# sony/DiffRoll

Measured on AMD Instinct MI355X. Metric: piano-roll frames/sec (200-step sample), higher is better.
Workload: dtype f32

## Files before the change

### diffroll_amd/csrc/abi.hip

```cpp
#include "engine_state.h"
#include "tenants.h"

#include <algorithm>
#include <condition_variable>
#include <mutex>

namespace drh {

thread_local std::string g_create_error;
void release_stager(int dev);
std::atomic<int> g_engines[MAX_DEVICES];

struct FusedSlot {
    std::mutex mu;
    std::condition_variable cv;
    dr_engine* owner = nullptr;
    bool claimed = false;
    hipEvent_t done = nullptr;
};
FusedSlot g_slots[MAX_DEVICES];

bool claim_fused_slot(dr_engine* e, hipStream_t st) {
    FusedSlot& s = g_slots[e->cfg.device];
    std::unique_lock<std::mutex> lk(s.mu);
// ... 377 lines not shown
        return DR_OK;
    }
    if (n == "start_noise") {
        if (value != 0 && value != 1)
            return fail(e, DR_EINVAL, "start_noise is 0 (x on entry is x at the start step) or 1 (a clean roll, diffused to it), got %d", value);
        e->opt.start_noise = value;
        return DR_OK;
    }
    if (n == "x0_clip") {
        if (value < 0 || value > 2)
            return fail(e, DR_EINVAL, "x0_clip is 0 (off), 1 (clamp the x0 prediction to [0, 1]) or 2 (to [-1, 1]), got %d", value);
        if (e->opt.x0_clamp != value) e->hist_key.valid = false;
        e->opt.x0_clamp = value;
        return DR_OK;
    }
    if (n == "x0_threshold") {
        if (value != 0 && (value < 5000 || value > 10000))
            return fail(e, DR_EINVAL, "x0_threshold is 0 (off) or the percentile in units of 1 / 10000, 5000 .. 10000 (9950 = 99.5 %%), got %d", value);
        if (e->opt.x0_thresh != value) e->hist_key.valid = false;
        e->opt.x0_thresh = value;
        return DR_OK;
    }
    if (n == "guidance_t_min" || n == "guidance_t_max") {
        const bool is_max = n == "guidance_t_max";
        if (!guidance_value_ok(is_max, value, e->S))
            return fail(e, DR_EINVAL, is_max ? "guidance_t_max is -1 (= timesteps - 1) or in [0, timesteps = %d), got %d"
                                             : "guidance_t_min is in [0, timesteps = %d), got %d", e->S, value);
        (is_max ? e->opt.guid.hi : e->opt.guid.lo) = value;
        return DR_OK;
    }
    if (!lab) return fail(e, DR_ENAME, "unknown option '%s'", name);
    if (n == "fused_stack_xcd") { if (e->opt_stack_xcd != value) drop(); e->opt_stack_xcd = value; return DR_OK; }
    if (n == "fused_stack_warm") { if (e->opt_stack_warm != value) drop(); e->opt_stack_warm = value; return DR_OK; }
#ifdef DR_FAULT_HOOK
    if (n == "stack_fault_test") { if (e->opt_stack_fault != value) drop(); e->opt_stack_fault = value; return DR_OK; }
#endif
    if (n == "stack_ticks") { if (e->stack_dbg_on != value) drop(); e->stack_dbg_on = value; return DR_OK; }
    if (n.compare(0, 5, "tune.") == 0) {
        Tuning& t = tuning();
        const std::string f = n.substr(5);
        if (f == "ksplit_blocks") {
            if (t.ksplit_blocks.load() != value) { t.ksplit_blocks.store(value); tuning_epoch().fetch_add(1); drop(); }
            return DR_OK;
        }
        std::atomic<int>* field = f == "pack_threads" ? &t.pack_threads : f == "tile" ? &t.tile : f == "pw" ? &t.pw : f == "pw_nw" ? &t.pw_nw
                   : f == "pwk" ? &t.pwk : f == "ksplit_max" ? &t.ksplit_max : f == "one_ks" ? &t.one_ks : f == "stack3" ? &t.stack3
                   : f == "stack_fl" ? &t.stack_fl : f == "tail_t4" ? &t.tail_t4 : f == "xcd_n" ? &t.xcd_n : f == "xcd_model" ? &t.xcd_model
                   : f == "s3_eager" ? &t.s3_eager : f == "debug_chunks" ? &t.debug_chunks : nullptr;
        if (!field) return fail(e, DR_ENAME, "unknown option '%s'", name);
        if (field->load() != value) {
            field->store(value);
            tuning_epoch().fetch_add(1);
            drop();
        }
        return DR_OK;
    }
    return fail(e, DR_ENAME, "unknown option '%s'", name);
}

int open_chain_call(dr_engine* e, int sampler, int B, int T, const int* step, int& NB, int& i0, hipStream_t st) {
    int rc = check_ready(e, sampler, B, T);
    if (rc) return rc;
    if (step) {
        const int t = *step;
        if (t < 0 || t >= e->S) return fail(e, DR_EINVAL, "step %d out of range", t);
        if (!e->rs_steps.empty() && std::find(e->rs_steps.begin(), e->rs_steps.end(), t) == e->rs_steps.end())
// ... 503 lines not shown
```

### diffroll_amd/csrc/engine_state.h

```cpp
#pragma once
#include <hip/hip_runtime.h>

#include <dlfcn.h>

#include <atomic>
#include <chrono>
#include <cmath>
#include <cstdarg>
#include <cstdio>
#include <cstdlib>
#include <cstring>
#include <map>
#include <memory>
#include <string>
#include <thread>
#include <vector>

#include "../../include/diffroll_amd_debug.h"
#include "device_buffer.h"
#include "fused_mode.h"
#include "kernels.h"

namespace drh {
using namespace dr;
// ... 113 lines not shown

    int ws_NB = 0, ws_T = 0;
    drh::DevBuf<float> sk_ws;
    drh::DevBuf<unsigned> sk_cnt;
    drh::DevBuf<float> h, hd, g, skip, tmp, x0buf;
    drh::DevBuf<float> xwork;
    drh::DevBuf<float> hd3, g3;
    int prec = 0;
    bool s3_ready = false;
    double t_pack_s = 0.0, t_upload_s = 0.0, t_tables_s = 0.0, t_capture_s = 0.0;
    int norm_framewise = 0;
    int fe_B = 0, fe_T = 0;
    drh::DevBuf<float> cond;
    drh::DevBuf<float> cond_dummy;
    drh::DevBuf<float> cond_tr;
    int cond_tr_T = 0;
    drh::DevBuf<float> wav_pad, power, logmel, specP4, mm;

    drh::GraphKey gkey;
    hipGraph_t graph = nullptr;
    hipGraphExec_t gexec = nullptr;
    drh::DevBuf<long long> dbg_ticks;
    drh::DevBuf<unsigned long long> d_counts;
    size_t mm_scratch_off = 0;
    hipStream_t cap_stream = nullptr;
    drh::DevBuf<dr::DynParams> d_dyn;
    drh::DevBuf<int> d_tsel;
    bool use_dyn = false;

    drh::FusedMode fused;
    int opt_stack_xcd = 1;
    int opt_stack_fault = 0;
    int opt_stack_warm = 0;
    int n_cus = 0;
    drh::StackSync sync;
    int opt_tail = 1;
    int64_t tail_launches = 0;
    drh::ChainOptions opt;
    std::vector<int> win_marks;
    drh::DevBuf<unsigned> d_wintab;
    std::vector<int> rs_steps;
    drh::DevBuf<float> d_coef_rs;
    std::vector<float> h_solver;
    drh::DevBuf<float> d_solver;
    drh::DevBuf<float> hist;
    int hist_par = 0;
    struct { bool valid = false; int sampler = -1, B = 0, T = 0, t = -1; } hist_key;
    drh::DevBuf<unsigned> thresh_work;
    int64_t inproj_launches = 0;
    int64_t conv0_launches = 0;
    unsigned win_epoch = 0;
    drh::DevBuf<float> xalt;
    int last_mode = 0;
    unsigned tuning_epoch = 0;
    long kfd_gpu_id = -1;
    double last_tenant_scan_s = -1.0;
    hipStream_t graph_stream = nullptr;
    bool graph_stream_set = false;
    bool unverified = false;
    hipStream_t fused_stream = nullptr;
    int opt_blocked = 2;
    drh::DevBuf<float> xsave;
    drh::DevBuf<long long> stack_dbg;
    int stack_dbg_on = 0;
    int64_t stack_launches = 0;

// ... 123 lines not shown
```

### diffroll_amd/csrc/gemm_body.h

```cpp
#pragma once
#include "device_common.h"

namespace dr {

DR_DEVINL void residual_quad(const float (&v)[4], const float4 bias, const float4 prev, float (&o)[4]) {
    float bb[4], pv[4];
    f4arr(bias, bb); f4arr(prev, pv);
#pragma unroll
    for (int e = 0; e < 4; ++e) o[e] = div_sqrt2(pv[e] + (v[e] + bb[e]));
}
DR_DEVINL void skip_quad(const float (&v)[4], const float4 bias, const float4 prev, const bool skip_init, float (&o)[4]) {
    float bb[4], pv[4];
    f4arr(bias, bb); f4arr(prev, pv);
#pragma unroll
    for (int e = 0; e < 4; ++e) o[e] = skip_init ? v[e] + bb[e] : (v[e] + bb[e]) + pv[e];
}
DR_DEVINL long cond_row(const GemmArgs& a, const int b) {
    int r = a.c_b0 + b;
    if (a.c_n > 0 && r >= a.c_n) r %= a.c_n;
    return r;
}
DR_DEVINL void gate_quad(const float (&v0)[4], const float (&v1)[4], const float4 bias0, const float4 bias1,
                         const float4 cond0, const float4 cond1, const bool has_c, float (&o)[4]) {
    float b0[4], b1[4], c0[4], c1[4];
// ... 16 lines not shown
DR_DEVINL void store_y2(const GemmArgs& a, const int b, const float (&o)[4], const float4 d, const int p0, const int t) {
    float o2[4];
    hd_quad(o, d, o2);
    if (a.out_s3 & 2) {
        store_s3_quad<COH3>(a.Y2 + (long)b * a.y2_bs, o2, p0, t, a.T, a.y_rows >> 3, a.wt_store);
    } else {
        float* dst2 = a.Y2 + (long)b * a.y2_bs + (long)(p0 >> 2) * a.y_ps + (long)t * a.y_fs;
        store_f4<COH4>(dst2, make_float4(o2[0], o2[1], o2[2], o2[3]), a.wt_store);
    }
}

DR_DEVINL AF4 load_a4(const __amdgpu_buffer_rsrc_t wrsrc, const int wvo, const int slab, const int NS, const int code) {
    AF4 o;
#pragma unroll
    for (int g = 0; g < 4; ++g) {
        DR_CHECK(slab >= 0 && wvo + slab * 16384 + g * 4096 + 16 <= NS * 16384, code, slab, NS);
        o.v[g] = buffer_load_f4(wrsrc, wvo, slab * 16384 + g * 4096);
    }
    return o;
}

typedef __attribute__((address_space(3))) void* lds_ptr;

template <int BN, int AUX, class PlaneOf>
DR_DEVINL void dma_tile(float4* Rs, PlaneOf plane_of, const int T, const int t0, const int first, const int stride, const int lane, const int code) {
    constexpr int RWL = (BN + 63) / 64;
    for (int i = first; i < 32 * RWL; i += stride) {
        const int pl = i / RWL, seg = i - pl * RWL;
        const int f = seg * 64 + lane;
        const __amdgpu_buffer_rsrc_t rsrc = __builtin_amdgcn_make_buffer_rsrc((void*)plane_of(pl), 0, (unsigned)T * 16u, 0x00020000);
        if (BN % 64 == 0 || f < BN) {
            DR_CHECK_LDS(Rs + pl * BN + f, lds_off(Rs), lds_off(Rs) + 32u * BN * 16u, code);
            __builtin_amdgcn_raw_ptr_buffer_load_lds(rsrc, (lds_ptr)(Rs + pl * BN + seg * 64), 16, (t0 + f) * 16, 0, 0, AUX);
        }
    }
}

template <int KS, int PREC, int AUX, int RBN>
DR_DEVINL void producer(const GemmArgs& a, float4* Xs, float4* Rs, const int pw, const int lane, const int mt, const int b, const int t0,
                        const int halo, const int FW, const int c0, const int c1, const int code_x, const int code_r) {
    constexpr int XP = (PREC ? 12 : 8) * KS;
    const int bx = a.x_bmod ? (b % a.x_bmod) : b;
    const float* Xg = a.X + (long)bx * a.x_bs;
    const int last_plane = a.x_planes - 1;
    const unsigned recs = ((unsigned)(a.T - 1) * (unsigned)a.x_fs + 4u) * 4u;
    const int wl = (FW + 63) >> 6;
    const int total = XP * wl;
    auto issue = [&](int chunk) {
        for (int i = pw; i < total; i += 4) {
            const int pl = i / wl, seg = i - pl * wl;
            const int f = seg * 64 + lane;
            const float* src;
            if constexpr (PREC) {
                const int sg = pl / 6, rem = pl - sg * 6, pce = rem >> 1, kq = rem & 1;
                const int pc = min(chunk * (4 * KS) + sg * 2 + kq, last_plane);
                src = Xg + (long)pce * a.x_piece + (long)pc * a.x_ps;
            } else {
                src = Xg + (long)min(chunk * XP + pl, last_plane) * a.x_ps;
            }
            const __amdgpu_buffer_rsrc_t rsrc = __builtin_amdgcn_make_buffer_rsrc((void*)src, 0, recs, 0x00020000);
            const int voff = (t0 - halo + f) * (int)a.x_fs * 4;
            float4* dst = Xs + (((chunk - c0) & 1) * XP + pl) * FW + seg * 64;
            if (f < FW) DR_CHECK_LDS(dst + lane, lds_off(Xs), lds_off(Xs) + 2u * XP * FW * 16u, code_x);
            if (f < FW) __builtin_amdgcn_raw_ptr_buffer_load_lds(rsrc, (lds_ptr)dst, 16, voff, 0, 0, AUX);
        }
    };
// ... 411 lines not shown
                        } else {
                            float* dst = a.skip + (long)be * a.s_bs + ((long)((p0 - a.y_rows) >> 2) * a.T + t) * 4;
                            skip_quad(v, ebias[q], eop[ni][q], a.skip_init, o);
                            *reinterpret_cast<float4*>(dst) = make_float4(o[0], o[1], o[2], o[3]);
                        }
                    } else {
                        if (p0 >= a.y_rows) continue;
                        float bb[4];
                        f4arr(ebias[q], bb);
    #pragma unroll
                        for (int e = 0; e < 4; ++e) {
                            if constexpr (EPI == EPI_PLAIN) o[e] = a.alpha * v[e] + bb[e];
                            else if constexpr (EPI == EPI_RELU) o[e] = fmaxf(a.alpha * v[e] + bb[e], 0.f);
                            else if constexpr (EPI == EPI_SILU) { const float z = v[e] + bb[e]; o[e] = z * sigmoidf_(z); }
                            else o[e] = logf(v[e] + 1e-6f);
                        }
                        float* dst = a.Y + (long)be * a.y_bs + (long)(p0 >> 2) * a.y_ps + (long)t * a.y_fs;
                        *reinterpret_cast<float4*>(dst) = make_float4(o[0], o[1], o[2], o[3]);
                        if constexpr (EPI == EPI_RELU) {
                            if (a.Y2) store_y2<COH, 0>(a, be, o, ed2[q], p0, t);
                        }
                    }
                }
            }
        }
    }
    if (a.dbg && blockIdx.x == 0 && tid == 0) {
        a.dbg[0] = tick1 - tick0;
        a.dbg[1] = clock64() - tick0;
    }
}

template <int NW, int COH, int RLDS, int TBN = 32 * NW, int EPI = EPI_RES_SKIP>
DR_DEVINL void pw_body(const GemmArgs& a, const int mt, const int nt, const int wave, float4* Rs = nullptr, const int foff = 0) {
    static_assert(EPI == EPI_RES_SKIP || EPI == EPI_RELU || EPI == EPI_PLAIN, "pw_body epilogues");
    static_assert(EPI == EPI_RES_SKIP || !RLDS, "the LDS-resident tile belongs to the residual / skip epilogue");
    constexpr int BN = TBN;
    int lane = threadIdx.x & 63;
    if constexpr (COH) asm volatile("" : "+v"(lane));
    const int r = lane & 31, hi = lane >> 5;
    const long long tick0 = a.dbg ? clock64() : 0;

    const int tps = (a.T + BN - 1) / BN;
    const int b = nt / tps;
    const int t0 = (nt % tps) * BN + foff;
    const int NS = a.kchunks;

    const __amdgpu_buffer_rsrc_t wr = __builtin_amdgcn_make_buffer_rsrc(
        (void*)(a.Wp + (long)mt * NS * 4096), 0, (unsigned)NS * 16384u, 0x00020000);
    const __amdgpu_buffer_rsrc_t xr = __builtin_amdgcn_make_buffer_rsrc(
        (void*)(a.X + (long)b * a.x_bs), 0, (unsigned)(a.x_planes * a.x_ps * 4), 0x00020000);
    const int wvo = (hi * 128 + wave * 32 + r) * 16;
    const int xps = (int)a.x_ps * 4;
    int xvo[NW];
#pragma unroll
    for (int ni = 0; ni < NW; ++ni) xvo[ni] = hi * xps + min(t0 + ni * 32 + r, a.T - 1) * 16;

    struct BF { float4 v[4][NW]; };
    auto load_a = [&](int slab) { return load_a4(wr, wvo, slab, NS, 120); };
    auto load_b = [&](int slab) -> BF {
        BF o;
#pragma unroll
        for (int g = 0; g < 4; ++g)
#pragma unroll
            for (int ni = 0; ni < NW; ++ni)
                o.v[g][ni] = buffer_load_f4(xr, xvo[ni], (slab * 8 + g * 2) * xps);
        return o;
// ... 36 lines not shown
        for (int q = 0; q < 4; ++q) {
            ebias[q] = *reinterpret_cast<const float4*>(a.bias + rowb + 8 * q);
            if constexpr (EPI == EPI_RES_SKIP)
                ed2[q] = *reinterpret_cast<const float4*>(a.d2 + (a.tsel ? (long)a.tsel[b] * a.d2_ts : 0) + min(rowb + 8 * q, a.y_rows - 4));
        }
        if constexpr (RLDS || EPI != EPI_RES_SKIP) return;
        const float* base = res_rows ? a.Y + (long)b * a.y_bs + (long)(rowb >> 2) * a.y_ps
                                     : a.skip + (long)b * a.s_bs + (long)((rowb - a.y_rows) >> 2) * a.T * 4;
        const long qs = res_rows ? 2 * a.y_ps : (long)2 * a.T * 4;
        const long fs = res_rows ? a.y_fs : 4;
#pragma unroll
        for (int ni = 0; ni < NW; ++ni) {
            const int tc = min(t0 + ni * 32 + r, a.T - 1);
#pragma unroll
            for (int q = 0; q < 4; ++q) eop[ni][q] = *reinterpret_cast<const float4*>(base + q * qs + tc * fs);
        }
    };
    int slab = 0;
    const int pre = max(NS - 2, 0) & ~1;
    for (; slab < pre; slab += 2) {
        step(std::false_type{}, slab);
        step(std::true_type{}, slab + 1);
        if (a.dbg && slab == 0 && blockIdx.x == 0 && threadIdx.x == 0) a.dbg[2] = clock64() - tick0;
    }
    if (a.dbg && blockIdx.x == 0 && threadIdx.x == 0) a.dbg[3] = clock64() - tick0;
    if constexpr (!RLDS) load_epilogue();
    __builtin_amdgcn_sched_barrier(0);
    for (; slab + 2 <= NS; slab += 2) {
        step(std::false_type{}, slab);
        step(std::true_type{}, slab + 1);
    }
    if (slab < NS) step(std::false_type{}, slab);
    const long long tick1 = a.dbg ? clock64() : 0;
    if constexpr (RLDS) load_epilogue();

#pragma unroll
    for (int ni = 0; ni < NW; ++ni) {
        const int t = t0 + ni * 32 + r;
        if (t >= a.T) continue;
#pragma unroll
        for (int q = 0; q < 4; ++q) {
            const int p0 = rowb + 8 * q;
            float v[4], o[4];
#pragma unroll
            for (int e = 0; e < 4; ++e) v[e] = acc[ni][4 * q + e];
            if constexpr (EPI != EPI_RES_SKIP) {
                if (p0 >= a.y_rows) continue;
                float bb[4];
                f4arr(ebias[q], bb);
#pragma unroll
                for (int e = 0; e < 4; ++e) {
                    o[e] = a.alpha * v[e] + bb[e];
                    if constexpr (EPI == EPI_RELU) o[e] = fmaxf(o[e], 0.f);
                }
                float* dst = a.Y + (long)b * a.y_bs + (long)(p0 >> 2) * a.y_ps + (long)t * a.y_fs;
                store_f4<COH>(dst, make_float4(o[0], o[1], o[2], o[3]), a.wt_store);
                continue;
            }
            float4* rs = nullptr;
            if constexpr (RLDS) rs = Rs + (wave * 8 + 2 * q + hi) * BN + foff + ni * 32 + r;
#ifdef DR_BOUNDS
            if constexpr (RLDS) DR_CHECK_LDS(rs, lds_off(Rs), lds_off(Rs) + 32u * BN * 16u, 121);
#endif
            float4 pv;
            if constexpr (RLDS) pv = *rs;
            else pv = eop[ni][q];
            if (res_rows) {
// ... 205 lines not shown
```

### diffroll_amd/csrc/kernels.h

```cpp
#pragma once
#include <hip/hip_runtime.h>
#include <stdint.h>

#include <atomic>

#include "launch_plan.h"

namespace dr {


struct Tuning {
    std::atomic<int> pack_threads{16};
    std::atomic<int> tile{0};
    std::atomic<int> pw{1};
    std::atomic<int> pw_nw{0};
    std::atomic<int> pwk{1};
    std::atomic<int> ksplit_max{16};
    std::atomic<long> ksplit_blocks{0};
    std::atomic<int> one_ks{0};
    std::atomic<int> stack3{1};
    std::atomic<int> stack_fl{0};
    std::atomic<int> tail_t4{0};
    std::atomic<int> xcd_n{-1};
    std::atomic<int> xcd_model{1};
// ... 49 lines not shown
    int wt_store;
};

hipError_t init_kernels();
hipError_t read_bounds(unsigned long long* out4);
hipError_t reset_bounds();
hipError_t launch_gemm(const GemmArgs& a, int epi, int NI, hipStream_t s, int prec = 0);
hipError_t launch_gemm16(const GemmArgs& a, int epi, int NJ, hipStream_t s);
hipError_t launch_pointwise(const GemmArgs& a, int NW, hipStream_t s);
hipError_t launch_pointwise_ksplit(const GemmArgs& a, int NW, hipStream_t s);

struct StackLayer {
    const float *conv_w, *conv_b, *conv_b2;
    const float *cond, *cond2;
    const float *out_w, *out_b;
    int dil, pad_;
};
struct StackArgs {
    float *h, *hd, *g, *skip;
    const float* d2;
    const int* tsel;
    long d2_ts;
    const float* zero;
    int NB, T, Cp, taps, n_cond, L;
    long c_bs;
    int c_b0, c_n;
    int p0, p1;
    int xcd_n;
    int rs_off;
    int lds_bytes;
    int fault;
    int fold128;
    int warm;
    unsigned* xid;
    unsigned* bar;
    unsigned* err;
    unsigned* derr;
    long long* dbg;
    StackLayer layer[DR_STACK_MAX_LAYERS];
};
hipError_t launch_stack(const StackArgs& s, int FL, int max_dil, hipStream_t st, int prec = 0);

struct DynParams {
    unsigned long long seed;
    int first_sample;
    float w, onepw;
    unsigned epoch;
};
hipError_t launch_set_dyn(DynParams* d, unsigned long long seed, int first_sample, float w, float onepw, unsigned epoch,
                          hipStream_t s);

struct UpdateArgs {
    float* x;
    const float* x0c;
    const float* x0u;
    const float* noise;
    const float* coef;
    int t;
    int mode;
    long n;
    long per_sample;
    float w, onepw;
    uint64_t seed;
    int first_sample;
    const DynParams* dyn;
    int win_H;
// ... 84 lines not shown
```

### diffroll_amd/csrc/launch_plan.h

```cpp
#pragma once
#include <algorithm>
#include <cstddef>

#include "../../include/diffroll_amd.h"

namespace dr {

enum Epilogue : int {
    EPI_PLAIN = 0,
    EPI_RELU = 1,
    EPI_SILU = 2,
    EPI_GATE = 3,
    EPI_RES_SKIP = 4,
    EPI_POWER = 5,
    EPI_LOG = 6
};

constexpr int DR_STACK_MAX_LAYERS = 30;
constexpr int STACK_GROUPS = 512;
constexpr size_t SK_WS_FLOATS = (size_t)16 << 20, SK_CNT_N = 4096;

struct PlanKnobs {
    int tile = 0, pw = 1, pw_nw = 0, pwk = 1, ksplit_max = 16;
    long ksplit_blocks = 0;
// ... 10 lines not shown

struct KSplitPlan { int ks; double us; double us_unsplit; };
inline KSplitPlan plan_ksplit(const PlanKnobs& k, long tiles, int nchunks, int kchunks, int taps, int NI, int prec,
                              size_t ws_floats, size_t ws_cnt_n) {
    const int ks_max = k.ksplit_max;
    const long forced_blocks = k.ksplit_blocks;
    const long max_blocks = forced_blocks ? forced_blocks : (prec ? 256 : 2048);
    const int BN = gemm_block_frames(NI);
    const double t_full = (double)kchunks * taps * 16.0 * (BN / 32) * 69.0 / 2400.0;
    auto cost = [&](int ks) {
        return (double)((tiles * ks + 255) / 256) * t_full / ks + (ks > 1 ? 4.0 + ks : 0.0);
    };
    KSplitPlan p{1, cost(1), cost(1)};
    for (int ks = 2; ks <= ks_max && ks <= 16; ks *= 2) {
        if (tiles * ks > max_blocks || nchunks % ks != 0) break;
        if ((size_t)tiles * ks * 128 * BN > ws_floats || (size_t)tiles * 4 > ws_cnt_n) break;
        const double c = cost(ks);
        if (tiles * ks <= 256 || c < 0.97 * p.us) { p.us = std::min(p.us, c); p.ks = ks; }
    }
    return p;
}

inline int stack_tile_frames(int FL) { return FL == 5 ? 160 : 64 * FL; }
inline size_t stack3_lds_bytes(int FL, int taps, int max_dil) {
    return std::max(gemm_lds_bytes(FL, 1, taps, max_dil, 1, EPI_GATE), gemm_lds_bytes(1, 4, 1, 1, 1, EPI_RES_SKIP)) + 16;
}
inline int stack_group_blocks(int FL, int Cp, int T) {
    const int BN = stack_tile_frames(FL);
    return (Cp >> 6) * ((T + BN - 1) / BN);
}
inline size_t stack_lds_bytes(int FL, int taps, int max_dil) {
    const int BN = stack_tile_frames(FL), halo = ((taps - 1) / 2) * max_dil;
    return (size_t)2 * 8 * (BN + 2 * halo) * 16 + (size_t)32 * BN * 16 + 16;
}

struct Tile { int flavor, n; };

inline double split_cost(const PlanKnobs& k, long blocks, int bn, double pen, int MT, int taps) {
    const int nchunks = 2 * MT;
    const KSplitPlan p = plan_ksplit(k, blocks, nchunks, nchunks, taps, bn / 64, 0, SK_WS_FLOATS, SK_CNT_N);
    if (p.ks <= 1 || blocks * p.ks <= 256) return 1e30;
    const double us_per_frame = p.us_unsplit / ((double)((blocks + 255) / 256) * bn);
    return 1.05 * pen * p.us / us_per_frame;
}
inline Tile pick_tile(const PlanKnobs& k, int MT, int NB, int T, int taps, int dil, int prec, int epi, bool allow16,
                      bool wide32 = false) {
    const int forced = k.tile;
    const int halo = ((taps - 1) / 2) * dil;
    struct Cand { int flavor, n, bn; double pen; };
    const Cand cands[] = {{0, 2, 128, 1.0}, {0, 5, 160, 1.04}, {1, 5, 160, 1.04}, {0, 3, 96, 1.04}, {1, 3, 96, 1.04}, {0, 1, 64, 1.0}};
    auto feasible = [&](const Cand& c) {
        if (c.flavor == 1 && (!allow16 || prec != 0)) return false;
        if (c.flavor == 0 && (c.n == 3 || c.n == 5) && (!wide32 || prec != 0 || epi != EPI_GATE || taps == 1)) return false;
        const int ks = (taps == 1) ? 2 : 1;
        const size_t lds = (c.flavor == 0)
            ? gemm_lds_bytes(c.n, (taps == 1 && c.n == 1) ? 4 : ks, taps, dil, prec, epi)
            : (size_t)2 * 8 * ks * (c.bn + 2 * halo) * 16 + (epi == EPI_RES_SKIP ? (size_t)32 * c.bn * 16 : 0);
        return lds <= 160 * 1024;
    };
    if (forced) {
        const int ff = forced / 100 == 16 ? 1 : 0, fn = forced % 100;
        for (const Cand& c : cands)
            if (c.flavor == ff && c.n == fn && feasible(c)) return Tile{ff, fn};
    }
    Tile best{0, 1};
    double best_cost = 1e30;
// ... 125 lines not shown
```

### diffroll_amd/csrc/plan.hip

```cpp
#include "engine_state.h"

namespace drh {

hipError_t launch_tiled(const GemmArgs& a, int epi, Tile t, hipStream_t s, int prec) {
    if (t.flavor == 3) return launch_pointwise_ksplit(a, t.n, s);
    if (t.flavor == 2) return launch_pointwise(a, t.n, s);
    return t.flavor == 1 ? launch_gemm16(a, epi, t.n, s) : launch_gemm(a, epi, t.n, s, prec);
}
void allow_splitk(const dr_engine* e, GemmArgs& a) {
    a.ws = e->sk_ws; a.ws_cnt = e->sk_cnt;
    a.ws_floats = SK_WS_FLOATS; a.ws_cnt_n = SK_CNT_N;
}

const float* g_zero_vecs[MAX_DEVICES] = {};
const float* zero_vec() {
    int dev = 0;
    (void)hipGetDevice(&dev);
    return (dev >= 0 && dev < MAX_DEVICES) ? g_zero_vecs[dev] : nullptr;
}

GemmArgs p4_gemm(const float* Wp, const float* bias, int MT, const float* X, int planes, int NB, int T) {
    GemmArgs a{};
    a.d2 = zero_vec();
    a.Wp = Wp; a.bias = bias ? bias : zero_vec(); a.MT = MT;
// ... 84 lines not shown
    a.X = v.xin; a.x_bs = (long)T * 88; a.x_ps = 4; a.x_fs = 88; a.x_planes = 22; a.x_bmod = v.bmod;
    a.kchunks = 3; a.NB = v.NB; a.T = T; a.taps = 1; a.dil = 1; a.alpha = 1.f;
    p4_out(a, e->h, Cp / 4, T, Cp);
    a.d2 = e->d_dtab + (v.tsel ? 0 : (size_t)v.t * e->L * Cp);
    a.tsel = v.tsel; a.d2_ts = (long)e->L * Cp;
    if (e->prec) { a.Y2 = e->hd3; a.y2_bs = act_bs + act_bs / 2; a.out_s3 = 2; }
    else { a.Y2 = e->hd; a.y2_bs = act_bs; }
    allow_splitk(e, a);
    HIPCHK(e, launch_gemm(a, EPI_RELU, pick_ni(k, a.MT, v.NB, T, 1, 1), v.st));
    e->inproj_launches += 1;
    return DR_OK;
}

static int launch_stack_range(const Eval& v, const NetPlan& p, int p0, int p1) {
    dr_engine* e = v.e;
    const int Cp = e->Cp, L = e->L, T = v.T, prec = e->prec;
    const long act_n = (long)Cp * T, c_bs = (long)2 * Cp * T;
    int b0 = 0;
    for (int ck = 0; ck < p.stack_chunks; ++ck) {
        const int nb = v.NB / p.stack_chunks + (ck < v.NB % p.stack_chunks ? 1 : 0);
        StackArgs sa{};
        sa.h = e->h + b0 * act_n; sa.hd = e->hd + b0 * act_n; sa.g = e->g + b0 * act_n; sa.skip = e->skip + b0 * act_n;
        if (prec) { sa.hd = e->hd3 + b0 * (act_n + act_n / 2); sa.g = e->g3 + b0 * (act_n + act_n / 2); }
        sa.d2 = e->d_dtab + (v.tsel ? 0 : (size_t)v.t * L * Cp);
        sa.tsel = v.tsel ? v.tsel + b0 : nullptr; sa.d2_ts = (long)L * Cp;
        sa.zero = zero_vec();
        sa.NB = nb; sa.T = T; sa.Cp = Cp; sa.taps = e->K; sa.L = L;
        sa.n_cond = std::max(0, std::min(nb, v.n_cond - b0));
        sa.c_bs = c_bs;
        sa.c_b0 = b0 < v.n_cond ? b0 : 0; sa.c_n = e->fe_B;
        sa.p0 = p0; sa.p1 = p1;
        sa.xcd_n = e->opt_stack_xcd;
        sa.warm = e->opt_stack_warm;
        sa.fault = e->opt_stack_fault;
        sa.fold128 = e->opt_blocked >= 2;
        sa.bar = e->sync.bar(); sa.err = e->sync.err; sa.derr = e->sync.derr(); sa.xid = e->sync.xid();
        sa.dbg = e->stack_dbg_on ? e->stack_dbg : nullptr;
        for (int l = 0; l < L; ++l) {
            const LayerW& w = e->layers[l];
            StackLayer& y = sa.layer[l];
            y.conv_w = prec ? w.conv_w3 : w.conv_w; y.conv_b = w.conv_b;
            y.conv_b2 = v.zero_spec ? w.conv_b_z : w.conv_b_u;
            y.cond2 = nullptr;
            if (e->cond_tr && !v.zero_spec) { y.cond2 = e->cond_tr + (size_t)l * 2 * Cp * T; y.conv_b2 = w.conv_b; }
            y.cond = e->cond ? e->cond + (size_t)l * e->fe_B * 2 * Cp * T : e->cond_dummy;
            y.out_w = prec ? w.out_w3 : w.out_w; y.out_b = w.out_b; y.dil = w.dil;
        }
        int rc = profiled(e, v.st, true, [&]() -> int {
            HIPCHK(e, launch_stack(sa, p.stack_fl, e->max_dil, v.st, prec));
            e->stack_launches += 1;
            e->unverified = true; e->fused_stream = v.st;
            return DR_OK;
        }, [&] {
            const double C = e->C, fr = (double)nb * T;
            for (int q = p0; q < p1; ++q)
                e->prof_flops += fr * 2.0 * C * 2.0 * C * ((q & 1) ? (q == 2 * L - 1 ? 0.5 : 1.0) : (double)e->K);
            e->prof_name = "stack_kernel<" + std::to_string(p.stack_fl) + "> (fused residual stack: dilated conv k=" +
                           std::to_string(e->K) + " + conditioner + gate and 1x1 + residual/skip, phases " +
                           std::to_string(p0) + ".." + std::to_string(p1 - 1) + " of " + std::to_string(2 * L) +
                           (p.stack_chunks > 1 ? ", " + std::to_string(p.stack_chunks) + " sample chunks" : "") +
                           (prec ? (p.fold ? ", split-bf16, blocked accumulation" : ", split-bf16, one chain per output")
                                 : (p.fold ? ", blocked accumulation" : ", one fp32 chain per output")) + ")";
        });
        if (rc) return rc;
        b0 += nb;
    }
// ... 256 lines not shown
```

### diffroll_amd/csrc/stack.hip

```cpp
#include "gemm_body.h"
#include "persistent.h"

namespace dr {

DR_BOUNDS_TU(stack)

template <int FL, int FOLDP = 1, int PREC = 0>
__global__ __launch_bounds__(512) void stack_kernel(const StackArgs s_by_value) {
    extern __shared__ __attribute__((aligned(16))) char smem[];
    (void)s_by_value;
    typedef const __attribute__((address_space(4))) StackArgs* KernArgs;
    const KernArgs sp = (KernArgs)__builtin_amdgcn_kernarg_segment_ptr();
    const __attribute__((address_space(4))) StackArgs& s = *sp;
    static_assert(FL == 1 || FL == 2 || (FL == 5 && FOLDP == 1 && PREC == 0), "block flavours");
    constexpr int BN = FL == 5 ? 160 : 64 * FL;
    constexpr int RP = 32;
    constexpr int RWL = (BN + 63) / 64;
    const int wave = __builtin_amdgcn_readfirstlane(threadIdx.x >> 6);
    const int MT = s.Cp >> 6;
    const int MB = MT;
    const int tps = (s.T + BN - 1) / BN;
    const unsigned gsize = (unsigned)(MB * tps);
    int mt, nt, grp, member;
    if (s.xcd_n) {
// ... 15 lines not shown
    unsigned episode = 0;
    float4* Rs = reinterpret_cast<float4*>(smem + s.rs_off);
    const int b_ = nt / tps, t0_ = (nt % tps) * BN;
    auto tile_plane = [&](int pl, bool& is_res) -> float* {
        const int row0 = mt * 128 + pl * 4;
        is_res = row0 < s.Cp;
        return is_res ? s.h + (long)b_ * act_bs + (long)(row0 >> 2) * s.T * 4
                      : s.skip + (long)b_ * act_bs + (long)((row0 - s.Cp) >> 2) * s.T * 4;
    };
    if constexpr (PREC) {
        if (pending_timeout) return;
    } else {
#ifdef DR_BOUNDS
        if (threadIdx.x == 0) DR_CHECK(s.rs_off + RP * BN * 16 + 16 <= s.lds_bytes && lds_off(smem) == 0u, 132, s.rs_off, s.lds_bytes);
#endif
        dma_tile<BN, 0>(Rs, [&](int pl) { bool is_res; return tile_plane(pl, is_res); }, s.T, t0_, wave, 8, threadIdx.x & 63, 131);
        if (pending_timeout) return;
        if (s.p0 & 1) {
            asm volatile("s_waitcnt vmcnt(0)" ::: "memory");
            __syncthreads();
        }
    }
    int wt_store = 1;
    unsigned my_tag = 0;
    unsigned& same_xcd_s = *reinterpret_cast<unsigned*>(Rs + RP * BN);
    if (threadIdx.x == 0) {
        unsigned my_xcc;
        asm volatile("s_getreg_b32 %0, hwreg(HW_REG_XCC_ID)" : "=s"(my_xcc));
        const unsigned gen = __hip_atomic_fetch_add(ctr + 2, 0u, __ATOMIC_RELAXED, __HIP_MEMORY_SCOPE_AGENT);
        my_tag = (gen << 4) | (my_xcc & 0xfu);
        __hip_atomic_store(s.xid + (long)grp * gsize + member, my_tag, __ATOMIC_RELAXED, __HIP_MEMORY_SCOPE_AGENT);
    }

#pragma unroll 1
    for (int p = s.p0; p < s.p1; ++p) {
        const int l = p >> 1;
        const __attribute__((address_space(4))) StackLayer& ly = sp->layer[l];
        if (s.dbg && blockIdx.x == 0 && threadIdx.x == 0) {
            s.dbg[p - s.p0] = clock64();
            if (p == s.p0) s.dbg[120] = wall_clock64();
        }
        GemmArgs a{};
        a.d2 = s.zero;
        a.lds_bytes = s.lds_bytes;
        a.wt_store = wt_store;
        a.MT = MT; a.NB = s.NB; a.T = s.T; a.alpha = 1.f; a.ksplit = 1;
        a.x_bs = act_bs; a.x_ps = (long)s.T * 4; a.x_fs = 4; a.x_planes = P; a.kchunks = s.Cp >> 5;
        a.y_bs = act_bs; a.y_ps = (long)s.T * 4; a.y_fs = 4; a.y_rows = s.Cp;
        if constexpr (PREC) {
            const long s3_bs = act_bs + act_bs / 2;
            if ((p & 1) == 0) {
                a.Wp = ly.conv_w; a.bias = ly.conv_b; a.bias2 = ly.conv_b2;
                a.X = s.hd; a.x_bs = s3_bs; a.x_piece = (long)(s.Cp >> 3) * s.T * 4; a.x_planes = s.Cp >> 3;
                a.taps = s.taps; a.dil = ly.dil;
                a.cond = ly.cond; a.cond2 = ly.cond2; a.c_bs = s.c_bs; a.c_b0 = s.c_b0; a.c_n = s.c_n; a.n_cond = s.n_cond;
                a.Y = s.g; a.y_bs = s3_bs; a.out_s3 = 1;
                gemm_body<FL, 1, EPI_GATE, 1, 1, FOLDP>(a, smem, mt, nt, 0);
            } else {
                a.Wp = ly.out_w; a.bias = ly.out_b;
                a.X = s.g; a.x_bs = s3_bs; a.x_piece = (long)(s.Cp >> 3) * s.T * 4; a.x_planes = s.Cp >> 3;
                a.taps = 1; a.dil = 1;
                a.Y = s.h;
                const bool last = (l + 1 == s.L);
                if (!last) {
                    a.Y2 = s.hd; a.y2_bs = s3_bs; a.out_s3 = 2;
                    a.d2 = s.d2 + (long)(l + 1) * s.Cp; a.tsel = s.tsel; a.d2_ts = s.d2_ts;
                }
                a.skip = s.skip; a.s_bs = act_bs; a.skip_init = (l == 0);
                const bool idle = last && mt < (s.Cp >> 7);
                const int tps64 = (s.T + 63) >> 6;
                const int b_ = nt / tps, ti = nt % tps;
#pragma unroll 1
                for (int half = 0; half < BN / 64; ++half) {
                    const int t64 = ti * (BN / 64) + half;
                    if (half) {
                        asm volatile("s_waitcnt vmcnt(0)" ::: "memory");
                        __syncthreads();
                    }
                    if (!idle && t64 < tps64) gemm_body<1, 4, EPI_RES_SKIP, 1, 1>(a, smem, mt, b_ * tps64 + t64, 0);
                }
            }
        } else
        if ((p & 1) == 0) {
            a.Wp = ly.conv_w; a.bias = ly.conv_b; a.bias2 = ly.conv_b2;
            a.X = s.hd; a.taps = s.taps; a.dil = ly.dil;
            a.cond = ly.cond; a.cond2 = ly.cond2; a.c_bs = s.c_bs; a.c_b0 = s.c_b0; a.c_n = s.c_n; a.n_cond = s.n_cond;
            a.Y = s.g;
            if (s.dbg && p + 2 >= s.p1) a.dbg = s.dbg + 64;
            gemm_body<FL, 1, EPI_GATE, 0, 1, FOLDP>(a, smem, mt, nt, 0);
            if (wave == 4) __builtin_amdgcn_fence(__ATOMIC_ACQUIRE, "agent");
            if (wave >= 4 && s.warm) {
                const int be = nt / tps;
                if (be < s.n_cond)
                    l2_touch(ly.cond + cond_row(a, be) * s.c_bs + (long)mt * 32 * s.T * 4, (unsigned)(32 * s.T * 16), wave - 4, 4);
                l2_touch(ly.out_w + (long)mt * (s.Cp >> 5) * 4096, (unsigned)((s.Cp >> 5) * 16384), wave - 4, 4);
            }
        } else {
            a.Wp = ly.out_w; a.bias = ly.out_b;
            a.X = s.g; a.taps = 1; a.dil = 1;
            a.Y = s.h;
            const bool last = (l + 1 == s.L);
            if (!last) {
                a.Y2 = s.hd; a.y2_bs = act_bs;
                a.d2 = s.d2 + (long)(l + 1) * s.Cp; a.tsel = s.tsel; a.d2_ts = s.d2_ts;
            }
            a.skip = s.skip; a.s_bs = act_bs; a.skip_init = (l == 0);
            const bool idle = last && mt < (s.Cp >> 7);
            if (s.dbg && p + 3 == s.p1) a.dbg = s.dbg + 96;
            if constexpr (FL == 2) {
                if (!idle) pw_body<2, 1, 1, 128>(a, mt, nt, wave & 3, Rs, (wave >> 2) * 64);
            } else if constexpr (FL == 5) {
                if (!idle) {
                    if (wave < 4) pw_body<3, 1, 1, 160>(a, mt, nt, wave, Rs, 0);
                    else pw_body<2, 1, 1, 160>(a, mt, nt, wave - 4, Rs, 96);
                }
            } else {
                if (wave < 4 && !idle) pw_body<BN / 32, 1, 1>(a, mt, nt, wave, Rs);
            }
            if (wave >= 4 && s.warm && !last) {
                const __attribute__((address_space(4))) StackLayer& nx = sp->layer[l + 1];
                l2_touch(nx.conv_w + (long)mt * (s.Cp >> 5) * s.taps * 4096, (unsigned)(2 * s.taps * 16384), wave - 4, 4);
            }
        }
        if (p + 1 < s.p1) {
            group_barrier<false>(ctr, ++episode * (gsize + DR_FAULT_EXTRA(s)), s.err, s.derr);
            if (episode == 1) {
                if (threadIdx.x == 0) {
                    unsigned same = 1;
                    for (unsigned i = 0; i < gsize; ++i)
                        same &= (__hip_atomic_load(s.xid + (long)grp * gsize + i, __ATOMIC_RELAXED, __HIP_MEMORY_SCOPE_AGENT) == my_tag);
                    same_xcd_s = same;
                }
                __syncthreads();
                wt_store = __builtin_amdgcn_readfirstlane(same_xcd_s ? 0 : 1);
            }
        }
    }
    if (s.dbg && blockIdx.x == 0 && threadIdx.x == 0) {
        s.dbg[s.p1 - s.p0] = clock64();
        s.dbg[121] = wall_clock64();
    }
    if constexpr (!PREC) {
        asm volatile("s_waitcnt vmcnt(0)" ::: "memory");
        __syncthreads();
        const int lane = threadIdx.x & 63;
        for (int i = wave; i < RP * RWL; i += 8) {
            const int pl = i / RWL, seg = i - pl * RWL;
            bool is_res;
            float* dst = tile_plane(pl, is_res);
            const int t = t0_ + seg * 64 + lane;
#ifdef DR_BOUNDS
            if (seg * 64 + lane < BN) DR_CHECK_LDS(Rs + pl * BN + seg * 64 + lane, s.rs_off, s.rs_off + RP * BN * 16, 133);
#endif
            if (seg * 64 + lane < BN && t < s.T && (!is_res || s.p1 < 2 * s.L))
                *reinterpret_cast<float4*>(dst + (long)t * 4) = Rs[pl * BN + seg * 64 + lane];
        }
    }
    if (threadIdx.x == 0) {
        const unsigned left = __hip_atomic_fetch_add(ctr + 1, 1u, __ATOMIC_RELAXED, __HIP_MEMORY_SCOPE_AGENT);
        if (left == gsize - 1) {
            __hip_atomic_store(ctr, 0u, __ATOMIC_RELAXED, __HIP_MEMORY_SCOPE_AGENT);
            __hip_atomic_store(ctr + 1, 0u, __ATOMIC_RELAXED, __HIP_MEMORY_SCOPE_AGENT);
            __hip_atomic_fetch_add(ctr + 2, 1u, __ATOMIC_RELAXED, __HIP_MEMORY_SCOPE_AGENT);
        }
    }
}

hipError_t launch_stack(const StackArgs& s, int FL, int max_dil, hipStream_t st, int prec) {
    if (FL != 1 && FL != 2 && FL != 5) return hipErrorInvalidValue;
    if (prec && ((s.Cp & 127) || FL == 5)) return hipErrorInvalidValue;
    if (s.L < 1 || s.L > DR_STACK_MAX_LAYERS || s.p0 < 0 || s.p1 > 2 * s.L || s.p0 >= s.p1 || (s.Cp & 63)) return hipErrorInvalidValue;
    const int BN = stack_tile_frames(FL), MT = s.Cp >> 6, gsize = stack_group_blocks(FL, s.Cp, s.T);
    const size_t lds = prec ? stack3_lds_bytes(FL, s.taps, max_dil) : stack_lds_bytes(FL, s.taps, max_dil);
    if (lds > 160 * 1024) return hipErrorInvalidValue;
    StackArgs b = s;
    b.rs_off = (int)(lds - 16 - (size_t)32 * BN * 16);
    b.lds_bytes = (int)lds;
    const int NBp = xcd_padded_groups(s.NB, gsize, &b.xcd_n);
#ifdef DR_BOUNDS
    for (int l = 0; l < s.L; ++l) {
        GemmArgs g{};
        g.MT = MT; g.NB = s.NB; g.T = s.T; g.taps = s.taps; g.kchunks = s.Cp >> 5; g.y_rows = s.Cp;
        g.x_bs = g.y_bs = g.y2_bs = g.s_bs = (long)s.Cp * s.T; g.x_ps = g.y_ps = (long)s.T * 4; g.x_fs = g.y_fs = 4; g.x_planes = s.Cp >> 2;
        g.Wp = s.layer[l].conv_w; g.bias = s.layer[l].conv_b; g.bias2 = s.layer[l].conv_b2; g.X = s.hd; g.Y = s.g;
        g.cond = s.layer[l].cond; g.cond2 = s.layer[l].cond2; g.c_bs = s.c_bs; g.c_b0 = s.c_b0; g.c_n = s.c_n; g.n_cond = s.n_cond;
        check_gemm_extents(g, EPI_GATE, 0, "stack_kernel (conv phase)");
        g.taps = 1; g.Wp = s.layer[l].out_w; g.bias = s.layer[l].out_b; g.X = s.g; g.Y = s.h; g.Y2 = s.hd; g.skip = s.skip;
        check_gemm_extents(g, EPI_RES_SKIP, 0, "stack_kernel (1x1 phase)");
    }
    host_extent(s.bar, (size_t)4 * 512 * 4, "group counters", "stack_kernel");
    host_extent(s.xid, (size_t)1024 * 4, "tag words", "stack_kernel");
#endif
    (void)MT;
    const dim3 grid((unsigned)(gsize * NBp));
    if (prec) {
        if (FL == 1) hipLaunchKernelGGL((stack_kernel<1, 1, 1>), grid, dim3(512), lds, st, b);
        else if (s.fold128) hipLaunchKernelGGL((stack_kernel<2, 1, 1>), grid, dim3(512), lds, st, b);
        else hipLaunchKernelGGL((stack_kernel<2, 0, 1>), grid, dim3(512), lds, st, b);
        return hipGetLastError();
    }
    if (FL == 1) hipLaunchKernelGGL((stack_kernel<1>), grid, dim3(512), lds, st, b);
    else if (FL == 5) hipLaunchKernelGGL((stack_kernel<5>), grid, dim3(512), lds, st, b);
    else if (FL == 2 && s.fold128) hipLaunchKernelGGL((stack_kernel<2, 1>), grid, dim3(512), lds, st, b);
    else if (FL == 2) hipLaunchKernelGGL((stack_kernel<2, 0>), grid, dim3(512), lds, st, b);
    else return hipErrorInvalidValue;
    return hipGetLastError();
}
hipError_t init_stack_kernels() {
    return allow_max_lds(&stack_kernel<1>, &stack_kernel<2, 0>, &stack_kernel<5>, &stack_kernel<2, 1>,
                         &stack_kernel<1, 1, 1>, &stack_kernel<2, 0, 1>, &stack_kernel<2, 1, 1>);
// ... 4 lines not shown
```

Measured before the change: 2258.

## Split last 1x1 stack phase across half-skip tiles to balance final layer work

For the FL=2, non-precision stack kernel, the last phase (the final 1x1 output projection) is pulled out of the layer loop and run with a split. Blocks in the lower half of the channel tiles help the upper half by taking the second 64-frame half of a partner tile. They pre-DMA that partner's skip slice into LDS, and the partner stores its half of the skip tile early during the preceding conv phase. The final writeback is changed so each block writes back only its own half of the skip accumulator. The aim is to spread the last phase's epilogue and skip traffic more evenly and shorten the kernel tail, at the cost of extra cross-block coordination, extra global stores and loads, and tricky correctness rules around the skip buffer.

```diff
diff --git a/diffroll_amd/csrc/abi.hip b/diffroll_amd/csrc/abi.hip
--- a/diffroll_amd/csrc/abi.hip
+++ b/diffroll_amd/csrc/abi.hip
@@ -433,6 +433,7 @@
     if (!lab) return fail(e, DR_ENAME, "unknown option '%s'", name);
     if (n == "fused_stack_xcd") { if (e->opt_stack_xcd != value) drop(); e->opt_stack_xcd = value; return DR_OK; }
     if (n == "fused_stack_warm") { if (e->opt_stack_warm != value) drop(); e->opt_stack_warm = value; return DR_OK; }
+    if (n == "stack_split_last") { if (e->opt_stack_split != value) drop(); e->opt_stack_split = value; return DR_OK; }
 #ifdef DR_FAULT_HOOK
     if (n == "stack_fault_test") { if (e->opt_stack_fault != value) drop(); e->opt_stack_fault = value; return DR_OK; }
 #endif
diff --git a/diffroll_amd/csrc/engine_state.h b/diffroll_amd/csrc/engine_state.h
--- a/diffroll_amd/csrc/engine_state.h
+++ b/diffroll_amd/csrc/engine_state.h
@@ -169,6 +169,7 @@
     int opt_stack_xcd = 1;
     int opt_stack_fault = 0;
     int opt_stack_warm = 0;
+    int opt_stack_split = 1;
     int n_cus = 0;
     drh::StackSync sync;
     int opt_tail = 1;
diff --git a/diffroll_amd/csrc/gemm_body.h b/diffroll_amd/csrc/gemm_body.h
--- a/diffroll_amd/csrc/gemm_body.h
+++ b/diffroll_amd/csrc/gemm_body.h
@@ -72,6 +72,34 @@
         if (BN % 64 == 0 || f < BN) {
             DR_CHECK_LDS(Rs + pl * BN + f, lds_off(Rs), lds_off(Rs) + 32u * BN * 16u, code);
             __builtin_amdgcn_raw_ptr_buffer_load_lds(rsrc, (lds_ptr)(Rs + pl * BN + seg * 64), 16, (t0 + f) * 16, 0, 0, AUX);
+        }
+    }
+}
+
+template <int BN>
+DR_DEVINL void half_skip_store(const float4* Rs, float* plane0, const int T, const int t0, const int pw, const int write_through) {
+    static_assert(BN == 128, "the 128-frame flavour");
+    int lane = threadIdx.x & 63;
+    asm volatile("" : "+v"(lane));
+    const int t = t0 + 64 + lane;
+    for (int pl = pw; pl < 32; pl += 4) {
+        DR_CHECK_LDS(Rs + pl * BN + 64 + lane, lds_off(Rs), lds_off(Rs) + 32u * BN * 16u, 134);
+        if (t < T) store_f4<1>(plane0 + ((long)pl * T + t) * 4, Rs[pl * BN + 64 + lane], write_through);
+    }
+}
+template <int BN>
+DR_DEVINL void half_skip_dma(float4* Rs, const float* plane0, const int T, const int t0, const int wave) {
+    static_assert(BN == 128, "the 128-frame flavour");
+    int lane = threadIdx.x & 63;
+    asm volatile("" : "+v"(lane));
+    const int f0 = 64 + (wave >> 2) * 32;
+#pragma unroll
+    for (int q = 0; q < 8; ++q) {
+        const int pl = (wave & 3) * 8 + q;
+        const __amdgpu_buffer_rsrc_t rsrc = __builtin_amdgcn_make_buffer_rsrc((void*)(plane0 + (long)pl * T * 4), 0, (unsigned)T * 16u, 0x00020000);
+        if (lane < 32) {
+            DR_CHECK_LDS(Rs + pl * BN + f0 + lane, lds_off(Rs), lds_off(Rs) + 32u * BN * 16u, 135);
+            __builtin_amdgcn_raw_ptr_buffer_load_lds(rsrc, (lds_ptr)(Rs + pl * BN + f0), 16, (t0 + f0 + lane) * 16, 0, 0, 16);
         }
     }
 }
@@ -549,7 +577,8 @@
 }
 
 template <int NW, int COH, int RLDS, int TBN = 32 * NW, int EPI = EPI_RES_SKIP>
-DR_DEVINL void pw_body(const GemmArgs& a, const int mt, const int nt, const int wave, float4* Rs = nullptr, const int foff = 0) {
+DR_DEVINL void pw_body(const GemmArgs& a, const int mt, const int nt, const int wave, float4* Rs = nullptr, const int foff = 0,
+                       const bool drain = false) {
     static_assert(EPI == EPI_RES_SKIP || EPI == EPI_RELU || EPI == EPI_PLAIN, "pw_body epilogues");
     static_assert(EPI == EPI_RES_SKIP || !RLDS, "the LDS-resident tile belongs to the residual / skip epilogue");
     constexpr int BN = TBN;
@@ -652,7 +681,10 @@
     }
     if (slab < NS) step(std::false_type{}, slab);
     const long long tick1 = a.dbg ? clock64() : 0;
-    if constexpr (RLDS) load_epilogue();
+    if constexpr (RLDS) {
+        if (drain) asm volatile("s_waitcnt vmcnt(0)" ::: "memory");
+        load_epilogue();
+    }
 
 #pragma unroll
     for (int ni = 0; ni < NW; ++ni) {
diff --git a/diffroll_amd/csrc/kernels.h b/diffroll_amd/csrc/kernels.h
--- a/diffroll_amd/csrc/kernels.h
+++ b/diffroll_amd/csrc/kernels.h
@@ -105,6 +105,7 @@
     int fault;
     int fold128;
     int warm;
+    int split_last;
     unsigned* xid;
     unsigned* bar;
     unsigned* err;
diff --git a/diffroll_amd/csrc/launch_plan.h b/diffroll_amd/csrc/launch_plan.h
--- a/diffroll_amd/csrc/launch_plan.h
+++ b/diffroll_amd/csrc/launch_plan.h
@@ -66,6 +66,12 @@
 inline size_t stack_lds_bytes(int FL, int taps, int max_dil) {
     const int BN = stack_tile_frames(FL), halo = ((taps - 1) / 2) * max_dil;
     return (size_t)2 * 8 * (BN + 2 * halo) * 16 + (size_t)32 * BN * 16 + 16;
+}
+
+inline bool stack_split_last(int FL, int prec, int Cp, int L, int p0, int p1) {
+    if (FL != 2 || prec != 0 || Cp <= 0 || Cp % 128 != 0 || L < 1) return false;
+    if (p1 != 2 * L || p0 < 0 || p0 >= p1) return false;
+    return p0 <= 2 * L - 2 || L == 1;
 }
 
 struct Tile { int flavor, n; };
diff --git a/diffroll_amd/csrc/plan.hip b/diffroll_amd/csrc/plan.hip
--- a/diffroll_amd/csrc/plan.hip
+++ b/diffroll_amd/csrc/plan.hip
@@ -140,6 +140,7 @@
         sa.p0 = p0; sa.p1 = p1;
         sa.xcd_n = e->opt_stack_xcd;
         sa.warm = e->opt_stack_warm;
+        sa.split_last = e->opt_stack_split;
         sa.fault = e->opt_stack_fault;
         sa.fold128 = e->opt_blocked >= 2;
         sa.bar = e->sync.bar(); sa.err = e->sync.err; sa.derr = e->sync.derr(); sa.xid = e->sync.xid();
diff --git a/diffroll_amd/csrc/stack.hip b/diffroll_amd/csrc/stack.hip
--- a/diffroll_amd/csrc/stack.hip
+++ b/diffroll_amd/csrc/stack.hip
@@ -71,8 +71,9 @@
         __hip_atomic_store(s.xid + (long)grp * gsize + member, my_tag, __ATOMIC_RELAXED, __HIP_MEMORY_SCOPE_AGENT);
     }
 
+    constexpr bool SPLIT = FL == 2 && PREC == 0;
 #pragma unroll 1
-    for (int p = s.p0; p < s.p1; ++p) {
+    for (int p = s.p0; p < s.p1 - (SPLIT ? s.split_last : 0); ++p) {
         const int l = p >> 1;
         const __attribute__((address_space(4))) StackLayer& ly = sp->layer[l];
         if (s.dbg && blockIdx.x == 0 && threadIdx.x == 0) {
@@ -128,6 +129,10 @@
             if (s.dbg && p + 2 >= s.p1) a.dbg = s.dbg + 64;
             gemm_body<FL, 1, EPI_GATE, 0, 1, FOLDP>(a, smem, mt, nt, 0);
             if (wave == 4) __builtin_amdgcn_fence(__ATOMIC_ACQUIRE, "agent");
+            if constexpr (FL == 2 && PREC == 0) {
+                if (wave >= 4 && s.split_last && p + 2 == s.p1 && p > s.p0 && mt >= (MT >> 1))
+                    half_skip_store<BN>(Rs, s.skip + (long)b_ * act_bs + (long)(mt - (MT >> 1)) * 32 * s.T * 4, s.T, t0_, wave - 4, wt_store);
+            }
             if (wave >= 4 && s.warm) {
                 const int be = nt / tps;
                 if (be < s.n_cond)
@@ -175,6 +180,32 @@
             }
         }
     }
+    if constexpr (FL == 2 && PREC == 0) {
+        if (s.split_last) {
+            const int p = s.p1 - 1, l = s.L - 1;
+            const __attribute__((address_space(4))) StackLayer& ly = sp->layer[l];
+            if (s.dbg && blockIdx.x == 0 && threadIdx.x == 0) {
+                s.dbg[p - s.p0] = clock64();
+                if (p == s.p0) s.dbg[120] = wall_clock64();
+            }
+            GemmArgs a{};
+            a.d2 = s.zero;
+            a.lds_bytes = s.lds_bytes;
+            a.wt_store = wt_store;
+            a.MT = MT; a.NB = s.NB; a.T = s.T; a.alpha = 1.f; a.ksplit = 1;
+            a.x_bs = act_bs; a.x_ps = (long)s.T * 4; a.x_fs = 4; a.x_planes = P; a.kchunks = s.Cp >> 5;
+            a.y_bs = act_bs; a.y_ps = (long)s.T * 4; a.y_fs = 4; a.y_rows = s.Cp;
+            a.Wp = ly.out_w; a.bias = ly.out_b;
+            a.X = s.g; a.taps = 1; a.dil = 1;
+            a.Y = s.h;
+            a.skip = s.skip; a.s_bs = act_bs; a.skip_init = (l == 0);
+            if (s.dbg) a.dbg = s.dbg + 100;
+            const bool helper = mt < (MT >> 1);
+            const bool fetch = helper && !a.skip_init;
+            if (fetch) half_skip_dma<BN>(Rs, s.skip + (long)b_ * act_bs + (long)mt * 32 * s.T * 4, s.T, t0_, wave);
+            pw_body<1, 1, 1, 128>(a, helper ? mt + (MT >> 1) : mt, nt, wave & 3, Rs, (helper ? 64 : 0) + (wave >> 2) * 32, fetch);
+        }
+    }
     if (s.dbg && blockIdx.x == 0 && threadIdx.x == 0) {
         s.dbg[s.p1 - s.p0] = clock64();
         s.dbg[121] = wall_clock64();
@@ -187,11 +218,18 @@
             const int pl = i / RWL, seg = i - pl * RWL;
             bool is_res;
             float* dst = tile_plane(pl, is_res);
+            bool wb = !is_res || s.p1 < 2 * s.L;
+            if constexpr (FL == 2) {
+                if (s.split_last) {
+                    wb = is_res ? seg == 1 : seg == 0;
+                    if (is_res) dst = s.skip + (long)b_ * act_bs + (long)(mt * 32 + pl) * s.T * 4;
+                }
+            }
             const int t = t0_ + seg * 64 + lane;
 #ifdef DR_BOUNDS
             if (seg * 64 + lane < BN) DR_CHECK_LDS(Rs + pl * BN + seg * 64 + lane, s.rs_off, s.rs_off + RP * BN * 16, 133);
 #endif
-            if (seg * 64 + lane < BN && t < s.T && (!is_res || s.p1 < 2 * s.L))
+            if (seg * 64 + lane < BN && t < s.T && wb)
                 *reinterpret_cast<float4*>(dst + (long)t * 4) = Rs[pl * BN + seg * 64 + lane];
         }
     }
@@ -215,6 +253,7 @@
     StackArgs b = s;
     b.rs_off = (int)(lds - 16 - (size_t)32 * BN * 16);
     b.lds_bytes = (int)lds;
+    b.split_last = s.split_last && stack_split_last(FL, prec, s.Cp, s.L, s.p0, s.p1);
     const int NBp = xcd_padded_groups(s.NB, gsize, &b.xcd_n);
 #ifdef DR_BOUNDS
     for (int l = 0; l < s.L; ++l) {
```

Result: no change. 2265, median of 6 (+0.3%).
